# scottdbrown/minion-plasmid-consensus

Measured on AMD Instinct MI355X. Metric: aligned bases/sec pileup+consensus (1/2/4/8 GPU) and % HBM roofline, higher is better.
Workload: dtype u8; 1 GPU; C2 (BASELINE configs[1]): pUC19-size 2,686 bp plasmid, 100k reads per GPU, sense+antisense pileup; ref_len=2686, local_reads=100000, samples_per_gpu=2, cs_bytes_gpu0=63325630, parallelism=read-shardx1, batches_in_flight=3, parse_cus=192

## Files before the change

minion-plasmid-consensus_amd/csrc/mpc_kernels.hip:

```cpp
#include <hip/hip_runtime.h>

#include <algorithm>
#include <atomic>
#include <cstring>
#include <string>
#include <type_traits>
#include <vector>

#include "mpc.h"
#include "mpc_device.h"

#if defined(MPC_STAMPS) || defined(MPC_STAMPS_LEFT)
#define MPC_BF_STAMPS_ 1
#else
#define MPC_BF_STAMPS_ 0
#endif
#if defined(MPC_TUNING_OVERRIDES)
#define MPC_BF_TUNING_ 2
#else
#define MPC_BF_TUNING_ 0
#endif
#if defined(MPC_LDS_BASE_MODES) || defined(MPC_LAYOUT_GAPS) || defined(MPC_FLANK_WAVES) || \
    defined(MPC_FLANK_BLOCKS_MAX) || defined(MPC_FLANK_SMALL_BELOW)
#define MPC_BF_VARIANT_ 4
// ... 2125 lines not shown
    }
  int32_t* tmp = d.wo_erun + d.wo_cap;
  auto starts = [&](int64_t k) { return k == 0 || (key[k] >> 32) != (key[k - 1] >> 32); };
  for (int64_t k = threadIdx.x; k < n; k += blockDim.x) tmp[k] = starts(k) ? 1 : 0;
  __syncthreads();
  const int64_t npos = block_scan_excl(tmp, n, s_w);
  for (int64_t k = threadIdx.x; k < n; k += blockDim.x) {
    const bool st = starts(k);
    const int32_t p = st ? tmp[k] : tmp[k] - 1;
    if (st) { d.wo_pos[p].g = (int32_t)(key[k] >> 32); d.wo_pos[p].beg = (int32_t)k; }
    if (k == n - 1 || starts(k + 1)) d.wo_pos[p].end = (int32_t)(k + 1);
  }
  __syncthreads();
  for (int64_t p = threadIdx.x; p < npos; p += blockDim.x) {
    int32_t m = 0;
    for (int32_t e = d.wo_pos[p].beg; e < d.wo_pos[p].end; ++e) m += (int32_t)(key[e] & 3u) == kWoDown;
    d.wo_pos[p].nrun = m + 1;
    tmp[p] = m + 1;
  }
  __syncthreads();
  block_scan_excl(tmp, npos, s_w);
  for (int64_t p = threadIdx.x; p < npos; p += blockDim.x) {
    WoPos& P = d.wo_pos[p];
    const int32_t run0 = tmp[p];
    P.run0 = run0;
    for (int32_t j = 0; j < P.nrun; ++j) {
      WoRun z;
      z.M = 0; z.R = 0; z.hiR = 0; z.loR = 0; z.C[0] = z.C[1] = z.C[2] = z.C[3] = 0u;
      d.wo_run[run0 + j] = z;
    }
    int32_t j = 0;
    for (int32_t e = P.beg; e < P.end; ++e) {
      d.wo_erun[e] = j;
      int32_t L, type;
      if (sh) { const WoRec rc = all[1 + idx[e]]; L = rc.len; type = rc.type; }
      else { const WoEv ev = d.wo[idx[e]]; L = wo_len(d, ev); type = ev.type; }
      WoRun& R = d.wo_run[run0 + j];
      if (type == kWoDown) { R.R = L; ++j; }
      else if (L > R.M) R.M = L;
    }
  }
  if (threadIdx.x == 0) d.status[MPC_ST_WRAP_POS] = (uint32_t)npos;
}

__device__ void wo_cover_read(const Dev& d, int np, int64_t r);
__global__ __launch_bounds__(256) void K_wocover(Dev d) {
  const int np = (int)d.status[MPC_ST_WRAP_POS];
  if (np == 0) return;
  for (int64_t r = (int64_t)blockIdx.x * blockDim.x + threadIdx.x; r < d.N; r += (int64_t)gridDim.x * blockDim.x)
    wo_cover_read(d, np, r);
}
__device__ void wo_cover_read(const Dev& d, int np, int64_t r) {
  const int s = d.sample[r];
  const int64_t n = d.n_of[s], gb = d.gbase[s];
  const int pa = wo_lower(d.wo_pos, np, gb), pb = wo_lower(d.wo_pos, np, gb + n);
  if (pa == pb) return;
  const uint8_t* ref = d.ref + d.ref_off[s];
  auto hit = [&](int p, int code) {
    const WoPos P = d.wo_pos[p];
    int lo = P.beg, hi = P.end;
    while (lo < hi) {
      const int mid = (lo + hi) >> 1;
      if (wo_key_read(d.wo_key[mid]) < d.read_offset + r) lo = mid + 1; else hi = mid;
    }
    const int32_t j = lo < P.end ? d.wo_erun[lo] : P.nrun - 1;
    atomicAdd(&d.wo_run[P.run0 + j].C[code], 1u);
    if (d.wo_x) wo_cov(d)[P.run0 + j] = 1;
  };
  const int64_t b = d.cs_off[r], e = d.cs_off[r + 1];
  int64_t i = d.tstart[r], o0 = b, olen = 0;
  uint32_t op = 0;
  for (int64_t x = b;; ++x) {
    const bool end = x >= e;
    const uint32_t c = end ? 0u : d.cs[x];
    const bool sp = !end && (c == ':' || c == 'Z' || c == '+' || c == '-' || c == '*');
    if (!end && !sp) { ++olen; continue; }
    if (end || olen > 0) {
      if (op == ':') {
        int64_t m = 0;
        if (!py_int(d.cs + o0, olen, &m)) return;
        if (m < 0) m = 0;
        if (m > (1ll << 40)) m = 1ll << 40;
        const int64_t k0 = i < 0 ? 0 : i, k1 = i + m < n ? i + m : n;
        for (int p = k0 < k1 ? wo_lower(d.wo_pos, np, gb + k0) : pb; p < pb && d.wo_pos[p].g < gb + k1; ++p) {
          const int code = base_code_exact(ref[d.wo_pos[p].g - gb]);
          if (code >= 0) hit(p, code);
        }
        i += m;
      } else if (op == '*') {
        if (olen == 0) return;
        if (i >= 0 && i < n) {
          const int p = wo_lower(d.wo_pos, np, gb + i);
          if (p < pb && d.wo_pos[p].g == gb + i) {
            const int code = code_upper(d.cs[o0 + olen - 1]);
            if (code >= 0) hit(p, code);
          }
        }
        i += 1;
      } else if (op == '-') {
        i += olen;
      } else if (op != '+' && op != 'Z') {
        return;
      }
      if (i >= n) return;
    }
    if (end) break;
    op = c;
    o0 = x + 1;
    olen = 0;
  }
}

__global__ __launch_bounds__(256) void K_wofold(Dev d) {
  const int np = (int)d.status[MPC_ST_WRAP_POS];
  const int32_t* cov = wo_cov(d);
  for (int64_t p = (int64_t)blockIdx.x * blockDim.x + threadIdx.x; p < np; p += (int64_t)gridDim.x * blockDim.x) {
    const WoPos P = d.wo_pos[p];
    for (int32_t j = 0; j < P.nrun; ++j)
      if (cov[P.run0 + j] != 0 && d.wo_run[P.run0 + j].M < 1) d.wo_run[P.run0 + j].M = 1;
  }
}


template <bool WO>
__global__ __launch_bounds__(kGB) void K_layout(Dev d, uint32_t epoch) {
  __shared__ int32_t s_w[2][kGB / 64];
  __shared__ int64_t s_pre[2];
  const int64_t b = blockIdx.x;
  const int64_t nb = (d.G + kGB - 1) / kGB;
  const int64_t g = b * kGB + threadIdx.x;
  int32_t rc = 0, dv = 0;
  int32_t F = 1, wop = -1;
  int s = 0;
  int64_t p = 0;
  if (g < d.G) {
    const int64_t r0 = (int64_t)d.right_start[g] + g, r1 = (int64_t)d.right_start[g + 1] + g + 1;
    int32_t lo = 0, hi = 0;
    for (int64_t t = r0; t < r1; ++t) {
      d.hiR[t] = hi;
      const int32_t m = d.M[t];
      if (m - hi > lo) lo = m - hi;
      if (t + 1 < r1) {
        d.loR[t] = lo;
        const int32_t R = d.runR[t];
        if (R - lo > hi) hi = R - lo;
      }
    }
    const int32_t mr = d.maxR[g];
    if (mr - lo > hi) hi = mr - lo;
    d.lo_f[g] = lo;
    int lo_s = 0, hi_s = d.S - 1;
    while (lo_s < hi_s) {
      const int mid = (lo_s + hi_s + 1) >> 1;
      if (d.gbase[mid] <= g) lo_s = mid; else hi_s = mid - 1;
    }
    s = lo_s;
    p = g - d.gbase[s];
    if constexpr (WO) {
      const int np = (int)d.status[MPC_ST_WRAP_POS];
      const int k = wo_lower(d.wo_pos, np, g);
      if (p < d.n_of[s] && k < np && d.wo_pos[k].g == g) {
        const WoPos P = d.wo_pos[k];
        int32_t wl = 0, wh = 0;
        for (int32_t j = 0; j < P.nrun; ++j) {
          WoRun& R = d.wo_run[P.run0 + j];
          const int32_t c1 = (R.C[0] | R.C[1] | R.C[2] | R.C[3]) != 0u ? 1 : 0;
          const int32_t m = R.M > c1 ? R.M : c1;
          R.hiR = wh;
          if (m - wh > wl) wl = m - wh;
          if (j + 1 < P.nrun) {
            R.loR = wl;
            if (R.R - wl > wh) wh = R.R - wl;
          }
        }
        F = wl + wh;
        wop = k;
        d.wo_pos[k].lo = wl;
        d.wo_pos[k].F = F;
      }
    }
    rc = lo + hi + (p < d.n_of[s] ? F : 0);
    d.rowcnt[g] = rc;
    dv = d.diff[g];
  }
  const int w = threadIdx.x >> 6, l = lane();
  const int ir = wave_scan_i32(rc), id = wave_scan_i32(dv);
  if (l == 63) { s_w[0][w] = ir; s_w[1][w] = id; }
  __syncthreads();
  int32_t wr = 0, wd = 0, br = 0, bd = 0;
  for (int k = 0; k < kGB / 64; ++k) {
    if (k < w) { wr += s_w[0][k]; wd += s_w[1][k]; }
    br += s_w[0][k];
    bd += s_w[1][k];
  }
  const uint64_t tag = (uint64_t)(epoch & 0x3fffffffu) << 32;
  if (w == 0) {
    const int32_t own[2] = {br, bd};
    int64_t pre[2];
    lookback<2>(reinterpret_cast<uint64_t*>(d.bsum), b, tag, own, pre, &d.status[MPC_ST_FLAGS]);
    if (l == 0) { s_pre[0] = pre[0]; s_pre[1] = pre[1]; }
  }
  __syncthreads();
  const int64_t pre_r = s_pre[0], pre_d = s_pre[1];
  if (b == nb - 1 && threadIdx.x == 0) {
    const int64_t tot = pre_r + br;
    d.status[MPC_ST_ROWS_NEEDED] = (uint32_t)tot;
    if (tot > d.row_cap) atomicOr(&d.status[MPC_ST_FLAGS], DE_CAP);
  }
  if (g >= d.G) return;
  const int64_t rb = pre_r + wr + ir - rc;
  const int64_t dep = pre_d + wd + id;
  d.row_base[g] = (int32_t)rb;
  if (p == 0) d.srow[s] = (int32_t)rb;
  if (rb + rc > d.row_cap) return;
  const int64_t n = d.n_of[s];
  const int64_t nslots = (int64_t)rc - (p < n ? F : 0);
  if (nslots > 0) d.meta[rb] = 2;
  if (p < n) {
    const uint32_t* sb = d.sub + g * 4;
    const uint32_t s0 = sb[0], s1 = sb[1], s2 = sb[2], s3 = sb[3];
    const int64_t match = dep - (int64_t)s0 - s1 - s2 - s3;
    uint32_t c[4] = {s0, s1, s2, s3};
    uint32_t fl = 0;
    if (match < 0) fl |= DE_INTERNAL;
    else if (match > 0) {
      const int rcode = base_code_exact(d.ref[d.ref_off[s] + p]);
      if (rcode < 0) fl |= DE_KEY;
      else c[rcode] += (uint32_t)match;
    }
    if (fl) atomicOr(&d.status[MPC_ST_FLAGS], fl);
    if (WO && wop >= 0) d.wo_pos[wop].row0 = (int32_t)(rb + nslots);
    else reinterpret_cast<uint4*>(d.rows)[rb + nslots] = make_uint4(c[0], c[1], c[2], c[3]);
    d.meta[rb + nslots] = 3;
  }
}


struct InsArgs {
  uint32_t* status; const int32_t* sample; const int32_t* gbase;
  int64_t read_offset, ovf_cap, G;
  const int32_t* right_start; const int32_t* rsl; const int32_t* roff; const int32_t* vals_out;
  const int32_t* row_base; const int32_t* lo_f; const int32_t* hiR;
  uint32_t* rows; const Ovf* ovf; const uint32_t* ovf_cnt; const uint8_t* cs;
  uint32_t* runt;
};

__global__ __launch_bounds__(kUB) void K_ins(InsArgs a) {
  const int l = lane();
  const int w = uniform_i32((int)(threadIdx.x >> 6));
  const bool cap = (a.status[MPC_ST_FLAGS] & DE_CAP) != 0;
  const bool no_ovf = *a.ovf_cnt == 0;
  const int64_t nwaves = (int64_t)gridDim.x * (blockDim.x >> 6);
  for (int64_t gw = (int64_t)w * gridDim.x + blockIdx.x; gw * 64 < a.G; gw += nwaves) {
    const int64_t g = gw * 64 + l;
    if (g >= a.G) continue;
    const int64_t t0 = (int64_t)a.right_start[g] + g + a.roff[g], t1 = t0 + (a.rsl[g + 1] - a.rsl[g]) + 1;
    const int64_t top = (int64_t)a.row_base[g] + a.lo_f[g] - 1;
    const bool excl = no_ovf && t1 - t0 == 1;
    for (int64_t t = t0; t < t1; ++t) {
      uint4* rt = reinterpret_cast<uint4*>(a.runt + t * 16);
      uint4 v[4];
#pragma unroll
      for (int bi = 0; bi < 4; ++bi) v[bi] = rt[bi];
#pragma unroll
      for (int bi = 0; bi < 4; ++bi) rt[bi] = make_uint4(0u, 0u, 0u, 0u);
      if (cap) continue;
      const int64_t rtop = top + a.hiR[t];
#pragma unroll
      for (int bi = 0; bi < 4; ++bi) {
        uint32_t* row = a.rows + (rtop - bi) * 4;
        if (excl) {
          if (v[bi].x | v[bi].y | v[bi].z | v[bi].w) *reinterpret_cast<uint4*>(row) = v[bi];
          continue;
        }
        if (v[bi].x) atomicAdd(row + 0, v[bi].x);
        if (v[bi].y) atomicAdd(row + 1, v[bi].y);
        if (v[bi].z) atomicAdd(row + 2, v[bi].z);
        if (v[bi].w) atomicAdd(row + 3, v[bi].w);
      }
    }
  }
  if (cap) return;
  const int64_t nov = *a.ovf_cnt < (uint32_t)a.ovf_cap ? *a.ovf_cnt : a.ovf_cap;
  for (int64_t t = (int64_t)blockIdx.x * (kUB / 64) + w; t < nov; t += (int64_t)gridDim.x * (kUB / 64)) {
    const Ovf o = a.ovf[t];
    const int64_t g = a.gbase[a.sample[o.read]] + o.gap;
    const int64_t run = run_left(a.right_start, a.rsl, a.roff, a.vals_out, g, a.read_offset + o.read);
    const int64_t rb = (int64_t)a.row_base[g] + a.lo_f[g] + a.hiR[run] - 1;
    for (int64_t bi = l; bi < o.len; bi += 64) {
      const int c = code_upper(a.cs[o.off + o.len - 1 - bi]);
      atomicAdd(a.rows + (rb - bi) * 4 + (c < 0 ? 0 : c), 1u);
    }
  }
}

#ifndef MPC_FLANK_WAVES
#define MPC_FLANK_WAVES 8
#endif
constexpr int kFW = MPC_FLANK_WAVES;
constexpr int kFWSmall = 2;
constexpr int kWinRows = 256;
constexpr int kFSeg = 256;
constexpr int kFStageLd = 2;
constexpr int kFStage = kFStageLd * 1024 - 16;
#ifndef MPC_FLANK_BLOCKS_MAX
#define MPC_FLANK_BLOCKS_MAX 512
#endif

struct FlankArgs {
  uint32_t* status; const int32_t* sample; const int32_t* n_of; const int32_t* gbase;
  const int32_t* tstart; const int32_t* i_end;
  const int64_t* up_off; const uint8_t* up; const int64_t* down_off; const uint8_t* down;
  const int32_t* right_start; const int32_t* rsl; const int32_t* roff; const int32_t* vals_out; const int32_t* rpos;
  const int32_t* row_base; const int32_t* lo_f; const int32_t* hiR; const int32_t* loR;
  uint32_t* rows;
  int64_t N, read_offset;
};

__device__ __forceinline__ int code_exact(uint32_t c) {
  const uint32_t h = (c >> 1) & 3u;
  const uint32_t expect = (0x47544341u >> (8 * h)) & 0xffu;
  const int code = (int)(((h & 1u) << 1) | (h >> 1));
  return c == expect ? code : -1;
}

__device__ __forceinline__ int32_t flank_gap(const FlankArgs& a, int64_t r, int side) {
  const int64_t* off = side ? a.down_off : a.up_off;
  if (off[r + 1] <= off[r]) return -1;
  const int s = a.sample[r];
  const int x = side ? a.i_end[r] : a.tstart[r];
  return (x >= 0 && x <= a.n_of[s]) ? a.gbase[s] + x : -1;
}

template <int NW, bool MULTI>
__global__ __launch_bounds__(NW * 64) __attribute__((amdgpu_waves_per_eu(MULTI || NW < kFW ? 4 : 6))) void K_flank(FlankArgs a) {
  __shared__ uint32_t win[2][kWinRows * 5];
  __shared__ __attribute__((aligned(16))) uint32_t own[NW][kFSeg];
  __shared__ __attribute__((aligned(16))) uint8_t stg[NW][2][kFStageLd * 64 * 16];
  __shared__ int64_t s_w0[2], s_wn[2][2];
  if (a.status[MPC_ST_FLAGS] & (DE_CAP | DE_INTERNAL)) return;
  const int tid = threadIdx.x, l = lane();
  const int w = uniform_i32(tid >> 6);
  const int64_t tot = a.status[MPC_ST_ROWS_NEEDED];
  constexpr int64_t RB = NW * 64;
  for (int k = tid; k < 2 * kWinRows * 5; k += blockDim.x) (&win[0][0])[k] = 0;
  const int64_t nchunks = (a.N + RB - 1) / RB;
  const int64_t cpb = MULTI ? (nchunks + gridDim.x - 1) / gridDim.x : 1;
  const int64_t ck0 = (int64_t)blockIdx.x * cpb, ck1 = ck0 + cpb < nchunks ? ck0 + cpb : nchunks;
  auto flush = [&]() {
    for (int side = 0; side < 2; ++side) {
      const int64_t w0 = s_w0[side];
      for (int k = tid; k < kWinRows * 4; k += blockDim.x) {
        const uint32_t v = win[side][(k >> 2) * 5 + (k & 3)];
        if (v) atomicAdd(a.rows + w0 * 4 + k, v);
      }
    }
  };
  uint32_t lerr = 0;
  int64_t lread = INT64_MAX;
  uint32_t* ow_w = own[w];
#pragma unroll 1
  for (int64_t ck = ck0; ck < ck1; ++ck) {
    if (tid < 2) {
      const int64_t c0 = ck * RB;
      const int64_t nr = a.N - c0 < RB ? a.N - c0 : RB;
      const int32_t x = flank_gap(a, c0, tid), y = flank_gap(a, c0 + nr / 2, tid), z = flank_gap(a, c0 + nr - 1, tid);
      const int32_t gw = (x == y || x == z) ? x : y;
      s_wn[ck & 1][tid] = gw >= 0 ? (int64_t)a.row_base[gw] : (int64_t)INT32_MIN;
      if (ck == ck0) s_w0[tid] = s_wn[ck & 1][tid];
    }
    const int64_t rb = ck * RB + (int64_t)w * 64;
    const int64_t r = rb + l;
    const bool live = r < a.N;
    int64_t off0 = 0, off1 = 0;
    int32_t L0 = 0, L1 = 0, rw0 = -1, rw1 = -1;
    if (live) {
      const int s = a.sample[r], ts = a.tstart[r], ie = a.i_end[r];
      off0 = a.up_off[r];
      off1 = a.down_off[r];
      const int64_t ul = a.up_off[r + 1] - off0, dl = a.down_off[r + 1] - off1;
      const int n = a.n_of[s];
      const int64_t gb = a.gbase[s];
      if (ul > 0 && ts >= 0 && ts <= n) {
        const int64_t g = gb + ts;
        int64_t hi = 0;
        if (a.right_start[g + 1] > a.right_start[g])
          hi = a.hiR[run_left(a.right_start, a.rsl, a.roff, a.vals_out, g, a.read_offset + r)];
        const int64_t rs = (int64_t)a.row_base[g] + a.lo_f[g] + hi - ul;
        if (rs >= 0 && rs + ul > tot) lerr |= DE_INTERNAL;
        else rw0 = (int32_t)rs;
      }
      if (dl > 0 && ie >= 0 && ie <= n) {
        const int64_t g = gb + ie;
        int64_t lo_at = 0;
        if (a.right_start[g + 1] > a.right_start[g]) {
          const int64_t t = a.rpos[r];
          lo_at = a.loR[(int64_t)a.right_start[g] + g + a.roff[g] + (t - a.rsl[g])];
        }
        const int64_t rs = (int64_t)a.row_base[g] + a.lo_f[g] - lo_at;
        if (rs >= 0 && rs + dl > tot) lerr |= DE_INTERNAL;
        else rw1 = (int32_t)rs;
      }
      L0 = ul < INT32_MAX ? (int32_t)ul : INT32_MAX;
      L1 = dl < INT32_MAX ? (int32_t)dl : INT32_MAX;
    }
    __syncthreads();
    const int64_t* wn_ = s_wn[ck & 1];
    if (MULTI && (wn_[0] != s_w0[0] || wn_[1] != s_w0[1])) {
      flush();
      __syncthreads();
      for (int k = tid; k < 2 * kWinRows * 5; k += blockDim.x) (&win[0][0])[k] = 0;
      if (tid < 2) s_w0[tid] = wn_[tid];
      __syncthreads();
    }
    if (rb >= a.N) continue;
    const int last = a.N - 1 - rb < 63 ? (int)(a.N - 1 - rb) : 63;
    const int64_t Bw0 = readlane64(off0, 0), nb0 = readlane64(off0 + L0, last) - Bw0;
    const int64_t Bw1 = readlane64(off1, 0), nb1 = readlane64(off1 + L1, last) - Bw1;
    const int32_t xo0 = live ? (int32_t)(off0 - Bw0) : (int32_t)min(nb0, (int64_t)INT32_MAX);
    const int32_t xo1 = live ? (int32_t)(off1 - Bw1) : (int32_t)min(nb1, (int64_t)INT32_MAX);
    auto stage_load = [&](const uint8_t* src, int64_t B, int64_t nb, int64_t c0, uint4 (&v)[kFStageLd]) {
      const int64_t A = (B + c0) & ~(int64_t)15;
      const int64_t cnt = nb - c0 < kFStage ? nb - c0 : kFStage;
      const int n16 = (int)(((B + c0 - A) + cnt + 15) >> 4);
#pragma unroll
      for (int j = 0; j < kFStageLd; ++j)
        v[j] = l + 64 * j < n16 ? *reinterpret_cast<const uint4*>(src + A + 16 * (l + 64 * j)) : make_uint4(0u, 0u, 0u, 0u);
    };
    auto stage_store = [&](uint8_t* st, const uint4 (&v)[kFStageLd]) {
#pragma unroll
      for (int j = 0; j < kFStageLd; ++j) *reinterpret_cast<uint4*>(st + 16 * (l + 64 * j)) = v[j];
    };
    {
      uint4 v0[kFStageLd], v1[kFStageLd];
      if (nb0 > 0) stage_load(a.up, Bw0, nb0, 0, v0);
      if (nb1 > 0) stage_load(a.down, Bw1, nb1, 0, v1);
      if (nb0 > 0) stage_store(stg[w][0], v0);
      if (nb1 > 0) stage_store(stg[w][1], v1);
    }
#pragma unroll 1
    for (int side = 0; side < 2; ++side) {
      const uint8_t* src = side ? a.down : a.up;
      const int32_t L = side ? L1 : L0, frs = side ? rw1 : rw0, xo = side ? xo1 : xo0;
      const int64_t Bw = side ? Bw1 : Bw0, nb = side ? nb1 : nb0;
      if (nb <= 0) continue;
      const int32_t w032 = s_w0[side] >= 0 ? (int32_t)s_w0[side] : -(1 << 30);
      uint32_t* wn = win[side];
      uint8_t* st = stg[w][side];
      if (nb >= (1 << 30)) {
        const int64_t fo = live ? (side ? a.down_off[r] : a.up_off[r]) : 0;
        const int64_t fl = live ? (side ? a.down_off[r + 1] : a.up_off[r + 1]) - fo : 0;
        for (int64_t j = 0; frs >= 0 && j < fl; ++j) {
          const int code = code_exact(src[fo + j]);
          if (code < 0) { lerr |= DE_KEY; lread = r < lread ? r : lread; continue; }
          const int32_t row = (int32_t)(frs + j);
          const uint32_t wr = (uint32_t)(row - w032);
          if (wr < (uint32_t)kWinRows) atomicAdd(wn + wr * 5 + code, 1u);
          else atomicAdd(a.rows + (int64_t)row * 4 + code, 1u);
        }
        continue;
      }
      const int32_t rowoff = (live && frs >= 0) ? frs - xo : INT32_MIN;
      const bool ne = live && L > 0;
      const int nb32 = (int)nb;
      int carry = 0;
#pragma unroll 1
      for (int c0 = 0; c0 < nb32; c0 += kFStage) {
        if (c0 > 0) {
          uint4 v[kFStageLd];
          stage_load(src, Bw, nb, c0, v);
          stage_store(st, v);
        }
        wave_sync_lds();
        const int sh = (int)((Bw + c0) & 15);
        const int c1 = nb32 - c0 < kFStage ? nb32 : c0 + kFStage;
#pragma unroll 1
        for (int S = c0; S < c1; S += kFSeg) {
          *reinterpret_cast<uint4*>(ow_w + 4 * l) = make_uint4(0u, 0u, 0u, 0u);
          wave_sync_lds();
          if (ne && xo >= S && xo < S + kFSeg && xo < c1) ow_w[xo - S] = (uint32_t)(l + 1);
          wave_sync_lds();
#pragma unroll
          for (int k = 0; k < 4; ++k) {
            const int x = S + 64 * k + l;
            const int inc = max(wave_scan_max_i32((int)ow_w[64 * k + l]), carry);
            carry = wave_last_i32(inc);
            const int32_t q = __builtin_amdgcn_ds_bpermute(4 * max(inc - 1, 0), rowoff);
            if (x >= c1 || inc == 0) continue;
            const int32_t row = x + q;
            if (row < 0) continue;
            const int code = code_exact(st[sh + (x - c0)]);
            if (code < 0) {
              lerr |= DE_KEY;
              const int64_t rr = rb + inc - 1;
              lread = rr < lread ? rr : lread;
              continue;
            }
            const uint32_t wr = (uint32_t)(row - w032);
            if (wr < (uint32_t)kWinRows) atomicAdd(wn + wr * 5 + code, 1u);
            else atomicAdd(a.rows + (int64_t)row * 4 + code, 1u);
          }
        }
        wave_sync_lds();
      }
    }
  }
  __syncthreads();
  if (ck1 > ck0) flush();
  if (lerr) {
    atomicOr(&a.status[MPC_ST_FLAGS], lerr);
    if (lread != INT64_MAX) atomicMin(&a.status[MPC_ST_FIRST_READ], (uint32_t)lread);
  }
}

__global__ __launch_bounds__(256) void K_worows(Dev d) {
  const int np = (int)d.status[MPC_ST_WRAP_POS];
  if (np == 0 || (d.status[MPC_ST_FLAGS] & DE_CAP)) return;
  const int64_t n_ev = wo_listed(d);
  const int l = lane();
  const int64_t nwaves = (int64_t)gridDim.x * (blockDim.x >> 6);
  const int64_t gw = (int64_t)blockIdx.x * (blockDim.x >> 6) + (threadIdx.x >> 6);
  for (int64_t p = gw; p < np; p += nwaves) {
    const WoPos P = d.wo_pos[p];
    for (int32_t j = l; j < P.nrun; j += 64) {
      const WoRun R = d.wo_run[P.run0 + j];
      uint32_t* row = d.rows + ((int64_t)P.row0 + P.lo + R.hiR - 1) * 4;
#pragma unroll
      for (int c = 0; c < 4; ++c)
        if (R.C[c]) atomicAdd(row + c, R.C[c]);
    }
  }
  uint32_t err = 0;
  int64_t eread = INT64_MAX;
  for (int64_t e = gw; e < n_ev; e += nwaves) {
    int64_t own = d.wo_idx[e];
    if (d.wo_x) {
      const WoRec rc = wo_all(d)[1 + own];
      if (rc.shard != d.shard) continue;
      own = rc.ev;
    }
    const WoEv ev = d.wo[own];
    const WoPos P = d.wo_pos[wo_lower(d.wo_pos, np, ev.g)];
    const WoRun R = d.wo_run[P.run0 + d.wo_erun[e]];
    const int64_t L = wo_len(d, ev);
    const uint8_t* src = ev.type == kWoIns ? d.cs + ev.src
                       : ev.type == kWoUp  ? d.up + d.up_off[ev.read]
                                           : d.down + d.down_off[ev.read];
    for (int64_t bi = l; bi < L; bi += 64) {
      int code;
      int64_t slot;
      if (ev.type == kWoDown) {
        code = code_exact(src[bi]);
        slot = (int64_t)P.lo - R.loR + bi;
      } else {
        const uint32_t c = src[L - 1 - bi];
        code = ev.type == kWoIns ? code_upper(c) : code_exact(c);
        slot = (int64_t)P.lo + R.hiR - 1 - bi;
      }
      if (code < 0) {
        err |= DE_KEY;
        eread = ev.read < eread ? ev.read : eread;
        continue;
      }
      atomicAdd(d.rows + ((int64_t)P.row0 + slot) * 4 + code, 1u);
    }
  }
  if (err) {
    atomicOr(&d.status[MPC_ST_FLAGS], err);
    atomicMin(&d.status[MPC_ST_FIRST_READ], (uint32_t)eread);
  }
}

__device__ __forceinline__ int sample_of_row(const Dev& d, int64_t row) {
  int lo = 0, hi = d.S - 1;
  while (lo < hi) {
    const int mid = (lo + hi + 1) >> 1;
    if (d.srow[mid] <= row) lo = mid; else hi = mid - 1;
  }
  return lo;
}

constexpr int kSmpLds = 512;
__device__ __forceinline__ void load_sample_rows(const Dev& d, int32_t* srow) {
  for (int s = threadIdx.x; s < d.S && s < kSmpLds; s += blockDim.x) srow[s] = d.srow[s];
}
__device__ __forceinline__ int sample_of_row_lds(const Dev& d, const int32_t* srow, int64_t row) {
  if (d.S > kSmpLds) return sample_of_row(d, row);
  int lo = 0, hi = d.S - 1;
  while (lo < hi) {
    const int mid = (lo + hi + 1) >> 1;
    if (srow[mid] <= row) lo = mid; else hi = mid - 1;
  }
  return lo;
}

constexpr int kCRBig = 8;
constexpr int64_t kCallBlocksMax = 512;

__device__ __forceinline__ uint4 call_slot(uint4 cv, double gtf, uint32_t* total_out) {
  const uint32_t total = cv.x + cv.y + cv.z + cv.w;
  *total_out = total;
  if (total == 0) return make_uint4(0, 0, 0, 0);
  uint64_t k0 = ((uint64_t)cv.x << 2) | 0u, k1 = ((uint64_t)cv.y << 2) | 1u;
  uint64_t k2 = ((uint64_t)cv.z << 2) | 2u, k3 = ((uint64_t)cv.w << 2) | 3u;
  auto cx = [](uint64_t& a, uint64_t& b) {
    const uint64_t hi = a > b ? a : b, lo = a > b ? b : a;
    a = hi; b = lo;
  };
  cx(k0, k1); cx(k2, k3); cx(k0, k2); cx(k1, k3); cx(k1, k2);
  const uint32_t c0 = (uint32_t)(k0 >> 2), c1 = (uint32_t)(k1 >> 2), c2 = (uint32_t)(k2 >> 2), c3 = (uint32_t)(k3 >> 2);
  auto name = [](uint64_t k) -> uint32_t { return (0x47435441u >> (8 * (uint32_t)(k & 3u))) & 0xffu; };
  const uint32_t m = (c0 > 0) + (c1 > 0) + (c2 > 0) + (c3 > 0);
  const uint32_t tie0 = c0 * (1u + (c1 == c0) + (c2 == c0) + (c3 == c0));
  const uint32_t tie1 = c1 * ((c0 == c1) + 1u + (c2 == c1) + (c3 == c1));
  const bool one = m == 1 || c0 > c1;
  uint32_t base = one ? name(k0) : 'N';
  const uint32_t count = one ? c0 : tie0;
  const bool two = m == 2 || c1 > c2;
  const uint32_t base2 = m <= 1 ? 'X' : (two ? name(k1) : 'N');
  const uint32_t count2 = m <= 1 ? 0u : (two ? c1 : tie1);
  const uint32_t chrom1 = base;
  if ((double)count < gtf * (double)count2) base = 'N';
  return make_uint4(base | (chrom1 << 8) | (base2 << 16) | (1u << 24), count, count2, total);
}

template <int kCR>
__global__ __launch_bounds__(256) __attribute__((amdgpu_waves_per_eu(kCR > 1 ? 4 : 8))) void K_call(Dev d, int64_t R) {
  constexpr int kCB = 256 * kCR;
  __shared__ int32_t srow[kSmpLds];
  __shared__ int32_t s_blk[2], s_w[4];
  const bool cap = (d.status[MPC_ST_FLAGS] & DE_CAP) != 0;
  const int64_t need0 = cap ? 0 : (int64_t)d.status[MPC_ST_ROWS_NEEDED];
  const int64_t need = need0 < R ? need0 : R;
  load_sample_rows(d, srow);
  const int64_t b0 = (int64_t)blockIdx.x * kCB;
  __syncthreads();
  if (threadIdx.x < 2) {
    const int64_t rr = threadIdx.x == 0 ? b0 : (b0 + kCB < need ? b0 + kCB : need) - 1;
    s_blk[threadIdx.x] = rr >= 0 ? sample_of_row_lds(d, srow, rr) : 0;
  }
  uint4 cv[kCR];
  uint8_t mt[kCR];
#pragma unroll
  for (int k = 0; k < kCR; ++k) {
    const int64_t row = b0 + threadIdx.x + 256 * k;
    cv[k] = row < R ? reinterpret_cast<const uint4*>(d.rows)[row] : make_uint4(0, 0, 0, 0);
    mt[k] = row < R ? d.meta[row] : 0;
  }
#pragma unroll
  for (int k = 0; k < kCR; ++k)
    if (b0 + threadIdx.x + 256 * k >= need) { cv[k] = make_uint4(0, 0, 0, 0); mt[k] = 0; }
  __syncthreads();
  int32_t dep[kCR];
#pragma unroll
  for (int k = 0; k < kCR; ++k) {
    const int64_t row = b0 + threadIdx.x + 256 * k;
    uint32_t total = 0;
    const uint4 out = call_slot(cv[k], d.gtf, &total);
    if (row < R) reinterpret_cast<uint4*>(d.res)[row] = out;
    dep[k] = (total > 0 && (mt[k] & 2u)) ? (int32_t)total : -1;
  }
  for (int sb = s_blk[0]; sb <= s_blk[1]; ++sb) {
    int32_t mx = -1;
#pragma unroll
    for (int k = 0; k < kCR; ++k) {
      const int64_t row = b0 + threadIdx.x + 256 * k;
      if (dep[k] > mx && (s_blk[0] == s_blk[1] || sample_of_row_lds(d, srow, row) == sb)) mx = dep[k];
    }
    mx = wave_max(mx);
    __syncthreads();
    if (lane() == 0) s_w[threadIdx.x >> 6] = mx;
    __syncthreads();
    if (threadIdx.x == 0) {
      const int32_t m = max(max(s_w[0], s_w[1]), max(s_w[2], s_w[3]));
      if (m >= 0 && (uint32_t)m > __hip_atomic_load(d.maxdepth + sb, __ATOMIC_RELAXED, __HIP_MEMORY_SCOPE_AGENT))
        atomicMax(d.maxdepth + sb, (uint32_t)m);
    }
  }
}

__global__ __launch_bounds__(256) __attribute__((amdgpu_waves_per_eu(8))) void K_select(Dev d, int64_t R, uint32_t epoch) {
  __shared__ int32_t srow[kSmpLds];
  __shared__ uint32_t smd[kSmpLds];
  __shared__ int32_t s_w[4];
  __shared__ int64_t s_pre;
  load_sample_rows(d, srow);
  for (int s = threadIdx.x; s < d.S && s < kSmpLds; s += blockDim.x) smd[s] = d.maxdepth[s];
  const int64_t b = blockIdx.x;
  const int64_t nb = (R + kKB - 1) / kKB;
  const int64_t base = b * kKB + 4 * threadIdx.x;
  uint4 v[4];
#pragma unroll
  for (int k = 0; k < 4; ++k) v[k] = base + k < R ? reinterpret_cast<const uint4*>(d.res)[base + k] : make_uint4(0, 0, 0, 0);
  __syncthreads();
  int c = 0;
  uint32_t bits = 0;
#pragma unroll
  for (int k = 0; k < 4; ++k) {
    if (v[k].x >> 24) {
      const int s = sample_of_row_lds(d, srow, base + k);
      const double thr = (double)(s < kSmpLds ? smd[s] : d.maxdepth[s]) * d.mdf;
      if ((double)v[k].y > thr) { ++c; bits |= 1u << k; }
    }
  }
  const int w = threadIdx.x >> 6, l = lane();
  const int inc = wave_scan_i32(c);
  if (l == 63) s_w[w] = inc;
  __syncthreads();
  int32_t wpre = 0, bt = 0;
  for (int k = 0; k < 4; ++k) { wpre += k < w ? s_w[k] : 0; bt += s_w[k]; }
  const uint64_t tag = (uint64_t)(epoch & 0x3fffffffu) << 32;
  if (w == 0) {
    int64_t pr;
    lookback<1>(reinterpret_cast<uint64_t*>(d.ksum), b, tag, &bt, &pr, &d.status[MPC_ST_FLAGS]);
    if (l == 0) s_pre = pr;
  }
  __syncthreads();
  const int64_t pre = s_pre;
  int64_t pos = pre + wpre + inc - c;
#pragma unroll
  for (int k = 0; k < 4; ++k)
    if (bits & (1u << k)) {
      const uint4 x = v[k];
      reinterpret_cast<uint4*>(d.calls)[pos++] = make_uint4(x.x & 0xffffffu, x.y, x.z, x.w);
    }
  const int64_t b0 = b * kKB, all = pre + bt;
  for (int s = 0; s < d.S; ++s) {
    const int64_t rb = s < kSmpLds ? srow[s] : d.srow[s];
    if (rb >= b0 && rb < b0 + kKB && (rb - b0) / 4 == threadIdx.x) {
      int64_t q = pre + wpre + inc - c;
      for (int k = 0; k < (int)((rb - b0) & 3); ++k) q += (bits >> k) & 1u;
      d.ncalls[s] = (int32_t)q;
    }
    if (b == nb - 1 && threadIdx.x == 0 && rb >= nb * kKB) d.ncalls[s] = (int32_t)all;
  }
  if (b == nb - 1 && threadIdx.x == 0) d.ncalls[d.S] = (int32_t)all;
}

}

static uint32_t next_epoch() {
  static std::atomic<uint32_t> e{0};
  uint32_t v;
  do v = (e.fetch_add(1) + 1) & 0x3fffffffu; while (v == 0);
  return v;
}

#define HIPCHK(x)                                                                  \
  do {                                                                             \
    hipError_t e_ = (x);                                                           \
    if (e_ != hipSuccess) return fail(MPC_E_HIP, std::string(#x) + ": " + hipGetErrorString(e_)); \
  } while (0)

template <class T>
static T* at(const mpc_plan* p, int b) { return reinterpret_cast<T*>(p->ws + p->off[b]); }

static Dev plan_dev(const mpc_plan* p) {
  using P = mpc_plan;
  const mpc_input& in = p->in;
  Dev d{};
  d.ref = in.ref; d.ref_off = in.ref_off; d.cs = in.cs; d.cs_off = in.cs_off; d.tstart = in.tstart;
  d.up = in.up; d.up_off = in.up_off; d.down = in.down; d.down_off = in.down_off; d.sample = in.sample;
  d.N = p->N; d.Ng = p->Ng; d.read_offset = in.read_offset; d.cs_base = in.cs_base; d.S = p->S; d.G = (int32_t)p->G;
  d.n_of = at<int32_t>(p, P::B_NOF); d.gbase = at<int32_t>(p, P::B_GBASE);
  d.status = at<uint32_t>(p, P::B_STATUS); d.i_end = at<int32_t>(p, P::B_IEND);
  d.ovf = at<Ovf>(p, P::B_OVF); d.ovf_cnt = at<uint32_t>(p, P::B_OVFCNT); d.ovf_cap = p->ovf_cap;
  d.hasleft = at<uint32_t>(p, P::B_HASLEFT); d.maxR = at<int32_t>(p, P::B_MAXR);
  d.keys_in = at<uint32_t>(p, P::B_KIN); d.vals_in = at<int32_t>(p, P::B_VIN);
  d.keys_out = at<uint32_t>(p, P::B_KOUT); d.vals_out = at<int32_t>(p, P::B_VOUT);
  d.keys_tmp = at<uint32_t>(p, P::B_KTMP); d.vals_tmp = at<int32_t>(p, P::B_VTMP);
  d.bcnt = at<int32_t>(p, P::B_BCNT); d.bpre = at<int32_t>(p, P::B_BPRE);
  d.gcnt = p->rsort_multi ? at<int32_t>(p, P::B_GCNT) : nullptr;
  d.kslot = p->rsort_multi ? at<int32_t>(p, P::B_KSLOT) : nullptr;
  d.rsflag = p->rsort_multi ? at<int32_t>(p, P::B_RSFLAG) : nullptr;
  d.rlen = at<int32_t>(p, P::B_RLEN); d.rpos = at<int32_t>(p, P::B_RPOS); d.right_start = at<int32_t>(p, P::B_RSTART);
  d.rsl = at<int32_t>(p, P::B_RSLOC); d.roff = at<int32_t>(p, P::B_ROFF); d.rcnt = at<int32_t>(p, P::B_RCNT);
  d.rcnt_all = at<int32_t>(p, P::B_RCNTALL); d.shard = p->shard; d.n_shards = p->n_shards;
  d.diff = at<int32_t>(p, P::B_DIFF); d.sub = at<uint32_t>(p, P::B_SUB);
  d.M = at<int32_t>(p, P::B_M); d.runR = at<int32_t>(p, P::B_RUNR); d.runt = at<uint32_t>(p, P::B_RUNT);
  d.hiR = at<int32_t>(p, P::B_HIR); d.loR = at<int32_t>(p, P::B_LOR);
  d.lo_f = at<int32_t>(p, P::B_LOF); d.rowcnt = at<int32_t>(p, P::B_ROWCNT); d.row_base = at<int32_t>(p, P::B_ROWBASE);
  d.bsum = at<int32_t>(p, P::B_BSUM);
  d.rows = at<uint32_t>(p, P::B_ROWS); d.meta = at<uint8_t>(p, P::B_META);
  d.row_cap = p->row_cap;
  d.res = at<uint32_t>(p, P::B_RES); d.keep = at<int32_t>(p, P::B_KEEP); d.ksum = at<int32_t>(p, P::B_KSUM);
  d.calls = at<uint32_t>(p, P::B_CALLS); d.ncalls = at<int32_t>(p, P::B_NCALLS); d.maxdepth = at<uint32_t>(p, P::B_MAXD);
  d.srow = at<int32_t>(p, P::B_SROW);
  d.wo = at<WoEv>(p, P::B_WOEV); d.wo_key = at<uint64_t>(p, P::B_WOKEY); d.wo_idx = at<uint32_t>(p, P::B_WOIDX);
  d.wo_erun = at<int32_t>(p, P::B_WOERUN); d.wo_pos = at<WoPos>(p, P::B_WOPOS); d.wo_run = at<WoRun>(p, P::B_WORUN);
  d.wo_cap = p->wo_cap;
  if (p->n_shards > 1 && p->wo_cap > 0) d.wo_x = at<uint8_t>(p, P::B_WOREC);
  return d;
}

// ... 406 lines not shown
```

Measured before the change: 3484 billion aligned bases/s.

## Derive flank window votes from per-lane loads and batch LDS reads in segment loop

Drops the serial flank_gap lookups done by two threads per chunk. The window-base vote now reuses the (gap, row_base) pairs each lane already loads, shared through LDS, which costs one extra __syncthreads per chunk. In the inner segment loop, all four ownership words and staged bytes are read from LDS up front, the four wave scans run back to back, and the bpermutes are batched, with asm barriers to keep that order. The goal is to hide LDS and cross-lane latency instead of serialising it per group, at the cost of more live registers.

```diff
diff --git a/minion-plasmid-consensus_amd/csrc/mpc_kernels.hip b/minion-plasmid-consensus_amd/csrc/mpc_kernels.hip
--- a/minion-plasmid-consensus_amd/csrc/mpc_kernels.hip
+++ b/minion-plasmid-consensus_amd/csrc/mpc_kernels.hip
@@ -2451,7 +2451,8 @@
 constexpr int kWinRows = 256;
 constexpr int kFSeg = 256;
 constexpr int kFStageLd = 2;
-constexpr int kFStage = kFStageLd * 1024 - 16;
+constexpr int kFStageBytes = kFStageLd * 64 * 16;
+constexpr int kFStage = kFStageBytes - 16;
 #ifndef MPC_FLANK_BLOCKS_MAX
 #define MPC_FLANK_BLOCKS_MAX 512
 #endif
@@ -2473,20 +2474,13 @@
   return c == expect ? code : -1;
 }
 
-__device__ __forceinline__ int32_t flank_gap(const FlankArgs& a, int64_t r, int side) {
-  const int64_t* off = side ? a.down_off : a.up_off;
-  if (off[r + 1] <= off[r]) return -1;
-  const int s = a.sample[r];
-  const int x = side ? a.i_end[r] : a.tstart[r];
-  return (x >= 0 && x <= a.n_of[s]) ? a.gbase[s] + x : -1;
-}
-
 template <int NW, bool MULTI>
 __global__ __launch_bounds__(NW * 64) __attribute__((amdgpu_waves_per_eu(MULTI || NW < kFW ? 4 : 6))) void K_flank(FlankArgs a) {
   __shared__ uint32_t win[2][kWinRows * 5];
   __shared__ __attribute__((aligned(16))) uint32_t own[NW][kFSeg];
-  __shared__ __attribute__((aligned(16))) uint8_t stg[NW][2][kFStageLd * 64 * 16];
+  __shared__ __attribute__((aligned(16))) uint8_t stg[NW][2][kFStageBytes];
   __shared__ int64_t s_w0[2], s_wn[2][2];
+  __shared__ int2 s_vote[2][3];
   if (a.status[MPC_ST_FLAGS] & (DE_CAP | DE_INTERNAL)) return;
   const int tid = threadIdx.x, l = lane();
   const int w = uniform_i32(tid >> 6);
@@ -2510,19 +2504,12 @@
   uint32_t* ow_w = own[w];
 #pragma unroll 1
   for (int64_t ck = ck0; ck < ck1; ++ck) {
-    if (tid < 2) {
-      const int64_t c0 = ck * RB;
-      const int64_t nr = a.N - c0 < RB ? a.N - c0 : RB;
-      const int32_t x = flank_gap(a, c0, tid), y = flank_gap(a, c0 + nr / 2, tid), z = flank_gap(a, c0 + nr - 1, tid);
-      const int32_t gw = (x == y || x == z) ? x : y;
-      s_wn[ck & 1][tid] = gw >= 0 ? (int64_t)a.row_base[gw] : (int64_t)INT32_MIN;
-      if (ck == ck0) s_w0[tid] = s_wn[ck & 1][tid];
-    }
     const int64_t rb = ck * RB + (int64_t)w * 64;
     const int64_t r = rb + l;
     const bool live = r < a.N;
     int64_t off0 = 0, off1 = 0;
     int32_t L0 = 0, L1 = 0, rw0 = -1, rw1 = -1;
+    int2 v0 = make_int2(-1, 0), v1 = make_int2(-1, 0);
     if (live) {
       const int s = a.sample[r], ts = a.tstart[r], ie = a.i_end[r];
       off0 = a.up_off[r];
@@ -2535,7 +2522,8 @@
         int64_t hi = 0;
         if (a.right_start[g + 1] > a.right_start[g])
           hi = a.hiR[run_left(a.right_start, a.rsl, a.roff, a.vals_out, g, a.read_offset + r)];
-        const int64_t rs = (int64_t)a.row_base[g] + a.lo_f[g] + hi - ul;
+        v0 = make_int2((int32_t)g, a.row_base[g]);
+        const int64_t rs = (int64_t)v0.y + a.lo_f[g] + hi - ul;
         if (rs >= 0 && rs + ul > tot) lerr |= DE_INTERNAL;
         else rw0 = (int32_t)rs;
       }
@@ -2546,12 +2534,27 @@
           const int64_t t = a.rpos[r];
           lo_at = a.loR[(int64_t)a.right_start[g] + g + a.roff[g] + (t - a.rsl[g])];
         }
-        const int64_t rs = (int64_t)a.row_base[g] + a.lo_f[g] - lo_at;
+        v1 = make_int2((int32_t)g, a.row_base[g]);
+        const int64_t rs = (int64_t)v1.y + a.lo_f[g] - lo_at;
         if (rs >= 0 && rs + dl > tot) lerr |= DE_INTERNAL;
         else rw1 = (int32_t)rs;
       }
       L0 = ul < INT32_MAX ? (int32_t)ul : INT32_MAX;
       L1 = dl < INT32_MAX ? (int32_t)dl : INT32_MAX;
+    }
+    {
+      const int64_t c0 = ck * RB;
+      const int64_t nr = a.N - c0 < RB ? a.N - c0 : RB;
+      if (r == c0) { s_vote[0][0] = v0; s_vote[1][0] = v1; }
+      if (r == c0 + nr / 2) { s_vote[0][1] = v0; s_vote[1][1] = v1; }
+      if (r == c0 + nr - 1) { s_vote[0][2] = v0; s_vote[1][2] = v1; }
+    }
+    __syncthreads();
+    if (tid < 2) {
+      const int2 x = s_vote[tid][0], y = s_vote[tid][1], z = s_vote[tid][2];
+      const int2 gw = (x.x == y.x || x.x == z.x) ? x : y;
+      s_wn[ck & 1][tid] = gw.x >= 0 ? (int64_t)gw.y : (int64_t)INT32_MIN;
+      if (ck == ck0) s_w0[tid] = s_wn[ck & 1][tid];
     }
     __syncthreads();
     const int64_t* wn_ = s_wn[ck & 1];
@@ -2629,16 +2632,34 @@
           wave_sync_lds();
           if (ne && xo >= S && xo < S + kFSeg && xo < c1) ow_w[xo - S] = (uint32_t)(l + 1);
           wave_sync_lds();
+          static_assert(15 + (kFStage - 1) / kFSeg * kFSeg + 191 < kFStageBytes, "groups 0-2 read inside the stage");
+          const int bx = sh + (S - c0) + l;
+          int o[4];
+          uint32_t ch[4];
+#pragma unroll
+          for (int k = 0; k < 4; ++k) o[k] = (int)ow_w[64 * k + l];
+#pragma unroll
+          for (int k = 0; k < 4; ++k) ch[k] = st[k < 3 ? bx + 64 * k : min(bx + 192, kFStageBytes - 1)];
+          asm volatile("" : "+v"(o[0]), "+v"(o[1]), "+v"(o[2]), "+v"(o[3]), "+v"(ch[0]), "+v"(ch[1]), "+v"(ch[2]), "+v"(ch[3]));
+#pragma unroll
+          for (int k = 0; k < 4; ++k) o[k] = wave_scan_max_i32(o[k]);
+          int32_t q[4];
+#pragma unroll
+          for (int k = 0; k < 4; ++k) {
+            const int top = wave_last_i32(o[k]);
+            o[k] = max(o[k], carry);
+            carry = max(top, carry);
+            q[k] = __builtin_amdgcn_ds_bpermute(4 * max(o[k] - 1, 0), rowoff);
+          }
+          asm volatile("" : "+v"(q[0]), "+v"(q[1]), "+v"(q[2]), "+v"(q[3]));
 #pragma unroll
           for (int k = 0; k < 4; ++k) {
             const int x = S + 64 * k + l;
-            const int inc = max(wave_scan_max_i32((int)ow_w[64 * k + l]), carry);
-            carry = wave_last_i32(inc);
-            const int32_t q = __builtin_amdgcn_ds_bpermute(4 * max(inc - 1, 0), rowoff);
+            const int inc = o[k];
             if (x >= c1 || inc == 0) continue;
-            const int32_t row = x + q;
+            const int32_t row = x + q[k];
             if (row < 0) continue;
-            const int code = code_exact(st[sh + (x - c0)]);
+            const int code = code_exact(ch[k]);
             if (code < 0) {
               lerr |= DE_KEY;
               const int64_t rr = rb + inc - 1;
```

Measured after the change: 3528 billion aligned bases/s (median of 6 runs). +1.3%, better.
